# google/ghost-dataplane

Hardware: AMD Instinct MI355X
Metric: Mpkt/s device-resident coprocessor NF pipeline (64B pkts); HBM GB/s vs peak (higher is better)
Workload: dtype u32

## Files before the change

ghost-dataplane_amd/csrc/cop_device.h:

```cpp
#ifndef COP_DEVICE_H
#define COP_DEVICE_H

#include <hip/hip_runtime.h>
#include <stdint.h>

#include "cop_kernels.h"

namespace copd {

constexpr int BLOCK = COPK_BLOCK;
constexpr int WAVES = BLOCK / 64;

typedef uint32_t u32x2 __attribute__((ext_vector_type(2)));
typedef uint32_t u32x4 __attribute__((ext_vector_type(4)));
typedef uint32_t u32x4a __attribute__((ext_vector_type(4), aligned(4)));
typedef uint32_t u32x2a __attribute__((ext_vector_type(2), aligned(4)));

__device__ __forceinline__ uint32_t bswap32(uint32_t x) { return __builtin_bswap32(x); }

__device__ __forceinline__ void lb_store(unsigned long long *p, unsigned long long v)
{
    __hip_atomic_store(p, v, __ATOMIC_RELAXED, __HIP_MEMORY_SCOPE_AGENT);
}

// ... 53 lines not shown
    for (uint32_t q = (uint32_t)wave; q < total; q += WAVES) {
        const bool b1 = q >= f1, b2 = q >= f2, b3 = q >= f3, b4 = q >= f4, b5 = q >= f5;
        const void *g = b5 ? s5.g : b4 ? s4.g : b3 ? s3.g : b2 ? s2.g : b1 ? s1.g : s0.g;
        uint32_t *dst = b5 ? s5.dst : b4 ? s4.dst : b3 ? s3.dst : b2 ? s2.dst : b1 ? s1.dst : s0.dst;
        const uint32_t n16 = b5 ? s5.n16 : b4 ? s4.n16 : b3 ? s3.n16 : b2 ? s2.n16 : b1 ? s1.n16 : s0.n16;
        const uint32_t c = q - (b5 ? f5 : b4 ? f4 : b3 ? f3 : b2 ? f2 : b1 ? f1 : 0u);
        const uint32_t i = c * 64u + (uint32_t)lane;
        if (i < n16)
            __builtin_amdgcn_global_load_lds((const __attribute__((address_space(1))) void *)((const uint4 *)g + i),
                                             (__attribute__((address_space(3))) void *)(dst + c * 256u), 16, 0, 0);
    }
}

__device__ __forceinline__ void lds_stage(uint32_t *lds_dst, const void *gsrc, uint32_t n16, int lane, int wave)
{
    const uint4 *g = (const uint4 *)gsrc;
    for (uint32_t c = (uint32_t)wave; c * 64u < n16; c += WAVES) {
        const uint32_t i = c * 64u + (uint32_t)lane;
        if (i < n16)
            __builtin_amdgcn_global_load_lds((const __attribute__((address_space(1))) void *)(g + i),
                                             (__attribute__((address_space(3))) void *)(lds_dst + c * 256u),
                                             16, 0, 0);
    }
}

__device__ __forceinline__ uint32_t ivt_search(const uint32_t *S, uint32_t m, uint32_t ib, uint32_t lv, uint32_t ip)
{
    const uint16_t *idx = (const uint16_t *)(S + m);
    const uint32_t b = ip >> (32u - ib);
    uint32_t k = idx[b];
    const uint32_t hi = idx[b + 1];
    for (uint32_t step = (1u << lv) >> 1; step; step >>= 1) {
        const uint32_t c = min(k + step, hi);
        if (S[c] <= ip) k = c;
    }
    return k;
}

#ifndef COPK_IVT_VALUE
#define COPK_IVT_VALUE 1
#endif
__device__ __forceinline__ uint32_t ivt_value(const uint32_t *S, const uint32_t *V, uint32_t m, uint32_t ib, uint32_t lv,
                                              uint32_t ip)
{
    if (!COPK_IVT_VALUE || lv == 0) return V[ivt_search(S, m, ib, lv, ip)];
    const uint16_t *idx = (const uint16_t *)(S + m);
    const uint32_t b = ip >> (32u - ib);
    uint32_t k = idx[b];
    const uint32_t hi = idx[b + 1];
    for (uint32_t step = (1u << lv) >> 1; step > 1; step >>= 1) {
        const uint32_t c = min(k + step, hi);
        if (S[c] <= ip) k = c;
    }
    const uint32_t c = min(k + 1, hi);
    const uint32_t sc = S[c], vk = V[k], vc = V[c];
    return sc <= ip ? vc : vk;
}

constexpr int LB_GROUPS = 4;
constexpr uint32_t LB_GAVE_UP = 0xFFFFFFFFu;
__device__ __forceinline__ uint32_t look_back(unsigned long long *chain, uint32_t stride, uint32_t j, uint32_t agg,
                                              uint32_t epoch, uint32_t *err, int lane, const uint32_t *exitw = nullptr,
                                              uint32_t spin_log2 = 22)
{
    const unsigned long long ep = (unsigned long long)epoch << 32;
    if (j == 0) {
        if (lane == 0) lb_store(&chain[0], ep | (2ull << 30) | agg);
        return 0;
    }
    if (lane == 0) lb_store(&chain[(size_t)j * stride], ep | (1ull << 30) | agg);
    uint32_t excl = 0;
    int qhi = (int)j - 1;
    uint32_t spins = 0;
    for (;;) {
        unsigned long long v[LB_GROUPS];
#pragma unroll
        for (int r = 0; r < LB_GROUPS; r++) {
            const int idx = qhi - r * 64 - lane;
            v[r] = idx >= 0 ? lb_load(&chain[(size_t)idx * stride]) : 0ull;
        }
        int consumed = 0;
        bool done = false;
#pragma unroll
        for (int r = 0; r < LB_GROUPS; r++) {
            const bool inb = qhi - r * 64 - lane >= 0;
            const uint32_t flag = (uint32_t)(v[r] >> 30) & 3u;
            const bool ok = inb && (uint32_t)(v[r] >> 32) == epoch && flag != 0u;
            const unsigned long long m_incl = __ballot(ok && flag == 2u);
            const unsigned long long m_bad = __ballot(inb && !ok);
            const int first_incl = m_incl ? __ffsll((long long)m_incl) - 1 : 64;
            const int first_bad = m_bad ? __ffsll((long long)m_bad) - 1 : 64;
            const int upto = min(first_incl + 1, first_bad);
            uint32_t val = lane < upto ? ((uint32_t)v[r] & 0x3FFFFFFFu) : 0u;
#pragma unroll
            for (int off = 32; off; off >>= 1) val += __shfl_xor(val, off);
            excl += val;
            consumed += upto;
            if (first_incl < first_bad) {
                done = true;
                break;
            }
            if (upto < 64) break;
        }
        if (done) break;
        qhi -= consumed;
        if (consumed == 0) {
// ... 157 lines not shown
__device__ __forceinline__ void load_step(const StepGeom &g, const uint8_t *pk0, uint32_t stride, uint32_t pb,
                                          uint32_t last, u32x4 (&v)[3], bool sys = false)
{
    if (sys) {
        const __amdgpu_buffer_rsrc_t rs = sys_rsrc(pk0);
#pragma unroll
        for (int c = 0; c < 3; c++) v[c] = ld_sys16(rs, min(pb + g.lpk[c], last) * stride + g.lch[c]);
        return;
    }
#pragma unroll
    for (int c = 0; c < 3; c++) {
        const uint32_t ic = min(pb + g.lpk[c], last);
        v[c] = __builtin_nontemporal_load((const u32x4 *)(pk0 + (size_t)ic * stride + g.lch[c]));
    }
}

__device__ __forceinline__ void load_step_imix(const StepGeom &g, const uint8_t *pkts, uint32_t off,
                                               uint32_t data_off, u32x4 (&v)[3], bool sys = false)
{
    uint32_t o[3];
#pragma unroll
    for (int c = 0; c < 3; c++)
        o[c] = (uint32_t)__builtin_amdgcn_ds_bpermute((int)(g.lpk[c] << 2), (int)off) + data_off + g.lch[c];
    if (sys) {
        const __amdgpu_buffer_rsrc_t rs = sys_rsrc(pkts);
#pragma unroll
        for (int c = 0; c < 3; c++) v[c] = ld_sys16(rs, o[c]);
        return;
    }
#pragma unroll
    for (int c = 0; c < 3; c++) v[c] = __builtin_nontemporal_load((const u32x4 *)(pkts + o[c]));
}

__device__ __forceinline__ uint32_t load_off_imix(const uint32_t *offsets, uint32_t pb, int lane, uint32_t last,
                                                  bool sys = false)
{
    const uint32_t ic = min(pb + (uint32_t)lane, last);
    return sys ? ld_sys4(sys_rsrc(offsets), ic * 4u) : offsets[ic];
}

__device__ __forceinline__ void gather_step(const StepGeom &g, const u32x4 (&v)[3], uint32_t &w3, uint32_t &w6,
                                            uint32_t &w7, uint32_t &w8)
{
    const uint32_t c0w = g.r3 == 0 ? v[0].w : g.r3 == 1 ? v[2].w : v[1].w;
    const uint32_t c1z = g.r3 == 0 ? v[1].z : g.r3 == 1 ? v[0].z : v[2].z;
    const uint32_t c1w = g.r3 == 0 ? v[1].w : g.r3 == 1 ? v[0].w : v[2].w;
    const uint32_t c2x = g.r3 == 0 ? v[2].x : g.r3 == 1 ? v[1].x : v[0].x;
    w3 = (uint32_t)__builtin_amdgcn_ds_bpermute(g.a3, (int)c0w);
    w6 = (uint32_t)__builtin_amdgcn_ds_bpermute(g.a67, (int)c1z);
    w7 = (uint32_t)__builtin_amdgcn_ds_bpermute(g.a67, (int)c1w);
    w8 = (uint32_t)__builtin_amdgcn_ds_bpermute(g.a8, (int)c2x);
}

struct Opt {
    uint32_t demux;
    uint32_t port_stats;
    uint32_t dbg;
    unsigned long long *rule_hits;
};

__device__ __forceinline__ Opt opt_all(const CopKParams &p)
{
    return Opt{p.demux, p.port_stats, p.dbg, p.rule_hits};
}

struct Tables {
    uint32_t *rt_top;
    uint16_t *rt_leaf;
    uint32_t *fw_s, *fw_v, *lp_s, *lp_v;
};

__device__ __forceinline__ uint32_t probe_ld(const uint32_t *a, uint32_t nt)
{
    return nt ? __builtin_nontemporal_load(a) : *a;
}

__device__ __forceinline__ void bkt_issue(const uint32_t *bidx, uint32_t ib, uint32_t ip, bool reach, uint32_t &k0,
                                          uint32_t &k1)
{
    if (reach) {
        const u32x2a x = *(const u32x2a *)(bidx + (ip >> (32u - ib)));
        k0 = x.x;
        k1 = x.y;
    } else {
        k0 = k1 = 0;
    }
}

template <int FW, int LPM, int PPT>
__device__ __forceinline__ void pass1(const CopKParams &p, const Tables &t, const uint32_t (&w3)[PPT],
                                      const uint32_t (&w6)[PPT], const uint32_t (&w7)[PPT],
                                      const uint32_t (&w8)[PPT], uint32_t (&verdict)[PPT], uint32_t (&port)[PPT],
                                      uint32_t (&src)[PPT], uint32_t (&dst)[PPT], uint32_t (&fwe)[PPT],
                                      uint32_t (&lpe)[PPT], uint32_t (&lpe2)[PPT], uint32_t (&fwe2)[PPT])
{
    const bool stageP = (p.stages & COPK_STAGE_PARSE) != 0;
#pragma unroll
    for (int k = 0; k < PPT; k++) {
        verdict[k] = COPK_FORWARD;
        port[k] = 0;
        const uint32_t et = ((w3[k] & 0xFFu) << 8) | ((w3[k] >> 8) & 0xFFu);
        dst[k] = bswap32(__builtin_amdgcn_alignbit(w8[k], w7[k], 16));
        src[k] = bswap32(__builtin_amdgcn_alignbit(w7[k], w6[k], 16));
        if (stageP) {
            if (et != 0x0800u) {
                verdict[k] = COPK_DROP_PARSE;
                port[k] = 0xFFFFu;
            } else {
                const uint32_t idx = dst[k] & 0xFFFFu;
                const uint32_t top = t.rt_top[idx >> 8];
                port[k] = (top & 0x80000000u) ? (uint32_t)t.rt_leaf[((top & 0xFFFFu) << 8) | (idx & 0xFFu)]
                                              : (top & 0xFFFFu);
                if (port[k] == 0xFFFFu) verdict[k] = COPK_DROP_PARSE;
                else if (port[k] >= p.n_ports) verdict[k] = COPK_DROP_NO_PORT;
            }
        }
        const bool reach = verdict[k] == COPK_FORWARD;
        if (FW == COPK_TBL_IVT) fwe[k] = ivt_value(t.fw_s, t.fw_v, p.fw_m, p.fw_ib, p.fw_lv, src[k]);
        if (FW == COPK_TBL_DIR) fwe[k] = reach ? probe_ld(&p.fw_tbl24[src[k] >> 8], p.probe_nt) : 0u;
        if (FW == COPK_TBL_BKT) bkt_issue(p.fw_bidx, p.fw_ib, src[k], reach, fwe[k], fwe2[k]);
        if (LPM == COPK_TBL_IVT) lpe[k] = ivt_value(t.lp_s, t.lp_v, p.lpm_m, p.lpm_ib, p.lpm_lv, dst[k]);
        if (LPM == COPK_TBL_DIR) lpe[k] = reach ? probe_ld(&p.lpm_tbl24[dst[k] >> 8], p.probe_nt) : 0u;
        if (LPM == COPK_TBL_TRIE) lpe[k] = t.lp_s[dst[k] >> 20];
        if (LPM == COPK_TBL_BKT) bkt_issue(p.lpm_bidx, p.lpm_ib, dst[k], reach, lpe[k], lpe2[k]);
    }
}

template <int PPT>
__device__ __forceinline__ void trie_walk(const uint32_t *nodes, const uint32_t *leaves, const uint32_t (&ip)[PPT],
                                          uint32_t (&e)[PPT], const bool (&live)[PPT])
{
    bool in[PPT], lf[PPT];
    bool any = false;
#pragma unroll
    for (int k = 0; k < PPT; k++) {
        in[k] = live[k] && (e[k] & 0x80000000u);
        lf[k] = false;
        any |= in[k];
    }
#pragma unroll
    for (int l = 0; l < 4; l++) {
        if (!__ballot(any)) break;
        const uint32_t sh = l == 0 ? 14u : l == 1 ? 8u : l == 2 ? 2u : 0u;
        const uint32_t msk = l == 3 ? 3u : 63u;
        u32x4a a[PPT];
        u32x2a b[PPT];
#pragma unroll
        for (int k = 0; k < PPT; k++) {
            if (in[k]) {
                const uint32_t *nd = nodes + (size_t)(e[k] & 0x7FFFFFFFu) * 6u;
                a[k] = *(const u32x4a *)nd;
                b[k] = *(const u32x2a *)(nd + 4);
            }
        }
        any = false;
#pragma unroll
        for (int k = 0; k < PPT; k++) {
            if (in[k]) {
                const uint32_t c = (ip[k] >> sh) & msk;
                const unsigned long long vec = a[k].x | ((unsigned long long)a[k].y << 32);
                const unsigned long long lv = a[k].z | ((unsigned long long)a[k].w << 32);
                const unsigned long long upto = (2ull << c) - 1ull;
                if ((vec >> c) & 1ull) {
                    e[k] = 0x80000000u | (b[k].x + (uint32_t)__popcll(vec & upto) - 1u);
                    any = true;
                } else {
                    e[k] = b[k].y + (uint32_t)__popcll(lv & upto) - 1u;
                    in[k] = false;
                    lf[k] = true;
                }
            }
        }
    }
#pragma unroll
    for (int k = 0; k < PPT; k++)
        if (lf[k]) e[k] = leaves[e[k]];
}

template <int PPT>
__device__ __forceinline__ void tbl8_step(const uint32_t *tbl8, uint32_t packed, const uint32_t (&ip)[PPT],
// ... 676 lines not shown
```

ghost-dataplane_amd/csrc/cop_runtime.cpp:

```cpp
#include <hip/hip_runtime.h>

#include <dlfcn.h>
#include <errno.h>
#include <stdarg.h>
#include <stdio.h>
#include <stdlib.h>
#include <string.h>
#include <time.h>

#include <algorithm>
#include <atomic>
#include <chrono>
#include <condition_variable>
#include <mutex>
#include <thread>
#include <vector>

#include "cop_gpu.h"
#include "cop_internal.h"
#include "cop_kernels.h"
#include <rccl/rccl.h>

namespace {

constexpr uint32_t IVT_MAX = 8192;
constexpr size_t SHARD_WORDS = (size_t)COPK_COUNTER_SHARDS * COP_N_COUNTERS;
constexpr size_t PORT_WORDS = (size_t)COPK_COUNTER_SHARDS * COPK_PORT_WORDS;
constexpr size_t RULE_OFF = SHARD_WORDS + PORT_WORDS;
constexpr uint32_t LOOK_TILE_MIN = COPK_BLOCK;
constexpr int TIMING_SLOTS = 256;
constexpr int MAX_LANES = 4;

struct DevLpm {
    bool loaded = false;
    uint32_t m = 0;
    uint32_t ib = 0, lv = 0, iw = 0;
    uint32_t *starts = nullptr, *vals = nullptr;
    uint32_t *tbl24 = nullptr, *tbl8 = nullptr;
    uint32_t n_ext = 0;
    bool tbl8_packed = false;
    size_t tbl8_bytes = 0;
    uint32_t *tl0 = nullptr, *tnodes = nullptr, *tleaves = nullptr;
    uint32_t t_nodes = 0, t_leaves = 0;
    uint32_t *bidx = nullptr, *bpairs = nullptr;
    uint32_t b_m = 0;
    cop_live_img *img = nullptr;
    uint64_t tab_uid = 0;
    uint32_t grp_cap = 0;
    bool has_table = false;
};

struct LookupStage {
    uint32_t *h = nullptr, *d = nullptr;
    hipEvent_t done = nullptr;
    uint32_t n = 0;
    uint64_t first = 0;
};

constexpr uint32_t LIVE_STAGE_RECS = 65536;
constexpr uint32_t IVT_IW_MAX = ((4096u + 2u) / 2u + 3u) & ~3u;
constexpr uint32_t IVT_STAGE_WORDS = 2 * IVT_MAX + IVT_IW_MAX;
struct LiveStage {
    cop_patch_rec *h = nullptr;
    void *d = nullptr;
    uint32_t *h_ivt = nullptr;
    hipEvent_t copied = nullptr;
    bool used = false;
};

struct Lane {
    hipStream_t s = nullptr;
    unsigned long long *tickets[2] = {nullptr, nullptr};
    uint32_t dirty[2] = {0, 0};
    int parity = 0;
// ... 1500 lines not shown
        L.zc = zc;
        if (zc_in) {
            HIPCHK(c, hipHostMalloc(&L.h_stage, (size_t)batch * COP_HDR16_STRIDE, hipHostMallocMapped));
            void *ds = nullptr;
            HIPCHK(c, hipHostGetDevicePointer(&ds, L.h_stage, 0));
            L.m_stage = (uint8_t *)ds;
        } else {
            HIPCHK(c, hipHostMalloc(&L.h_stage, (size_t)batch * COP_HDR16_STRIDE, hipHostMallocDefault));
            HIPCHK(c, hipMalloc(&L.d_stage, (size_t)batch * COP_HDR16_STRIDE));
        }
        if (zc_out) {
            HIPCHK(c, hipHostMalloc(&L.h_res, (size_t)batch * 8, hipHostMallocMapped));
            void *dr = nullptr;
            HIPCHK(c, hipHostGetDevicePointer(&dr, L.h_res, 0));
            L.m_res = (cop_result *)dr;
        } else {
            HIPCHK(c, hipHostMalloc(&L.h_res, (size_t)batch * 8, hipHostMallocDefault));
            HIPCHK(c, hipMalloc(&L.d_res, (size_t)batch * 8));
        }
        L.cap = batch;
    }
    const uint64_t nb = (n + batch - 1) / batch;
    const bool overlap = c->gather && c->gather->th.size() > 0 && c->n_lanes > 1;
    auto prepare = [&](uint64_t bi, bool async) -> int {
        Lane &L = c->lane[bi % (uint64_t)c->n_lanes];
        const uint64_t first = bi * batch;
        const uint32_t k = (uint32_t)std::min<uint64_t>(batch, n - first);
        const cop_result *prev = nullptr;
        uint32_t prev_n = 0;
        uint64_t prev_first = 0;
        if (L.busy) {
            HIPCHK(c, hipEventSynchronize(L.done));
            L.busy = false;
            prev = L.h_res;
            prev_n = L.n;
            prev_first = L.first;
        }
        cop_result *prev_dst = prev ? results + prev_first : nullptr;
        const size_t prev_bytes = (size_t)prev_n * sizeof(cop_result);
        if (c->gather && async) {
            c->gather->start_async(pkt_data + first, L.h_stage, k, prev, prev_dst, prev_bytes, rec);
        } else if (c->gather) {
            c->gather->run(pkt_data + first, L.h_stage, k, prev, prev_dst, prev_bytes, rec);
        } else {
            if (prev_n) memcpy(prev_dst, prev, prev_bytes);
            GatherPool::slice(pkt_data + first, L.h_stage, k, 1, 0, rec);
        }
        return 0;
    };
    auto issue = [&](uint64_t bi) -> int {
        Lane &L = c->lane[bi % (uint64_t)c->n_lanes];
        const uint64_t first = bi * batch;
        const uint32_t k = (uint32_t)std::min<uint64_t>(batch, n - first);
        if (!zc_in && !(c->dbg & 0x100u))
            HIPCHK(c, hipMemcpyAsync(L.d_stage, L.h_stage, (size_t)k * rec, hipMemcpyHostToDevice, L.s));
        cop_batch b;
        memset(&b, 0, sizeof(b));
        b.pkts = zc_in ? L.m_stage : L.d_stage;
        b.n = k;
        b.stride = rec;
        b.results = zc_out ? L.m_res : L.d_res;
        if (int rc = submit_on(c, L, &b, 1, false, c->cfg.stages)) return rc;
        if (!zc_out) HIPCHK(c, hipMemcpyAsync(L.h_res, L.d_res, (size_t)k * 8, hipMemcpyDeviceToHost, L.s));
        HIPCHK(c, hipEventRecord(L.done, L.s));
        L.busy = true;
        L.first = first;
        L.n = k;
        return 0;
    };
    if (nb)
        if (int rc = prepare(0, false)) return rc;
    for (uint64_t bi = 0; bi < nb; bi++) {
        const bool pre = overlap && bi + 1 < nb;
        if (pre)
            if (int rc = prepare(bi + 1, true)) return rc;
        const int rc = issue(bi);
        if (pre) c->gather->wait();
        if (rc) return rc;
        if (!overlap && bi + 1 < nb)
            if (int rc2 = prepare(bi + 1, false)) return rc2;
    }
    for (int l = 0; l < c->n_lanes; l++)
        if (int rc = lane_finish(c, c->lane[l], results)) return rc;
    if (int rc = take_lane_errors(c, 0xFu)) return rc;
    return 0;
}

static int pmd_hits_flush(cop_ctx *c);
static int pmd_pause(cop_ctx *c);
static int pmd_resume(cop_ctx *c);

static int tele_scratch(cop_ctx *c)
{
    HIPCHK(c, hipSetDevice(c->device));
    if (!c->tele_stream) HIPCHK(c, hipStreamCreateWithFlags(&c->tele_stream, hipStreamNonBlocking));
    const size_t n = RULE_OFF + c->n_rule_ctr;
    if (c->tele_words < n) {
        if (c->tele_dev) (void)hipFree(c->tele_dev);
        c->tele_dev = nullptr;
        c->tele_words = 0;
        HIPCHK(c, hipMalloc(&c->tele_dev, n * 8));
        c->tele_words = n;
    }
    return 0;
}

static int exchange_words(cop_ctx *c, size_t off, size_t n, uint64_t *out, int reset)
// ... 1807 lines not shown
```

ghost-dataplane_amd/csrc/cop_tile.h:

```cpp
#ifndef COP_TILE_H
#define COP_TILE_H

#include "cop_device.h"

namespace copd {

#ifndef COPK_PHASE_STAMPS
#define COPK_PHASE_STAMPS 0
#endif
#define STAMP(ph)                                                                          \
    do {                                                                                   \
        if (((o.dbg & 8u) || (COPK_PHASE_STAMPS && p.stamps)) && tid == 0) {               \
            __builtin_amdgcn_sched_barrier(0);                                             \
            __hip_atomic_store(&p.stamps[blockIdx.x * 8 + (ph)], __builtin_amdgcn_s_memrealtime(), \
                               __ATOMIC_RELAXED, __HIP_MEMORY_SCOPE_AGENT);                     \
            __builtin_amdgcn_sched_barrier(0);                                             \
        }                                                                                  \
    } while (0)

struct LdsCarve {
    Tables tb;
    CompactLds cl;
    uint32_t *s_tile;
    uint32_t *s_red;
// ... 157 lines not shown
#endif
#ifndef COPK_PMD_WIN
#define COPK_PMD_WIN 1
#endif
#ifndef COPK_PMD_WIN_DIR
#define COPK_PMD_WIN_DIR COPK_PMD_WIN
#endif
template <int PPT, int WIN>
constexpr int win_of()
{
    return WIN < PPT ? WIN : PPT;
}
#ifndef COPK_PMD_PRIO
#define COPK_PMD_PRIO 1
#endif
template <int K>
__device__ __forceinline__ void step_prio()
{
    if constexpr (COPK_PMD_PRIO) __builtin_amdgcn_s_setprio(K >= 3 ? 0 : 3 - K);
}
#ifndef COPK_PMD_PRIO_BODY
#define COPK_PMD_PRIO_BODY 0
#endif
template <bool WT, int K>
__device__ __forceinline__ void body_prio()
{
    if constexpr (WT && COPK_PMD_PRIO_BODY) step_prio<K>();
}
#ifndef COPK_PMD_STAGE_LIST
#define COPK_PMD_STAGE_LIST 1
#endif
#ifndef COPK_SEG_WAVE
#define COPK_SEG_WAVE 1
#endif
#ifndef COPK_WAVE_COUNTERS
#define COPK_WAVE_COUNTERS 1
#endif
template <int PPT>
__device__ __forceinline__ uint32_t step_off(int k, int wave)
{
    if constexpr (COPK_SEG_WAVE && PPT == WAVES) return (uint32_t)(wave * PPT * 64 + k * 64);
    else return (uint32_t)(k * BLOCK + wave * 64);
}

template <int PPT, int K0, int K1, int SYS = 2, int WIN = COPK_PMD_WIN>
__device__ __forceinline__ void steps_load(const CopKBatch &B, uint32_t j, int lane, int wave,
                                           u32x4 (&v)[win_of<PPT, WIN>()][3], bool sys_rt = false)
{
    const bool sys = SYS == 2 ? sys_rt : SYS == 1;
    static_assert(K1 <= win_of<PPT, WIN>(), "steps beyond the window");
    const StepGeom sg = step_geom(lane);
    const uint32_t base = j * (BLOCK * PPT);
    const uint32_t last = B.n ? B.n - 1 : 0u;
#pragma unroll
    for (int k = K0; k < K1; k++)
        load_step(sg, B.pkts + B.data_off, B.stride, base + step_off<PPT>(k, wave), last, v[k], sys);
}

template <int FW, int LPM, int PPT, bool WT, int SYS = 2, int WIN = COPK_PMD_WIN,
          bool STAGE_LIST = COPK_PMD_STAGE_LIST, int LAY = COPK_LAY_COALESCED>
__device__ __forceinline__ void tile_steps_v(const CopKParams &p, const LdsCarve &lc, const CopKBatch &B, uint32_t j,
                                             int tid, int lane, int wave, u32x4 (&v)[win_of<PPT, WIN>()][3],
                                             bool sys_rt = false)
{
    const bool sys = SYS == 2 ? sys_rt : SYS == 1;
    static_assert(COPK_SEG == BLOCK, "one segment per tile step");
    const Tables &tb = lc.tb;
    constexpr int TILE = BLOCK * PPT;
    const uint32_t base = j * TILE;
    const uint32_t last = B.n ? B.n - 1 : 0u;
    const StepGeom sg = step_geom(lane);
    constexpr int W = win_of<PPT, WIN>();
    Counts tot;
    uint32_t *r = (uint32_t *)B.results;
    const int i2 = lane & 31;
    const bool staged = STAGE_LIST && B.fwd_idx && lc.cl.stage && !(COPK_XP & 4);
    uint32_t all_prev = 0;
    auto flush = [&](int k, uint32_t len) {
        const uint32_t cc = (uint32_t)wave * 16u + (uint32_t)(lane & 15);
        const uint32_t pk = base + (uint32_t)k * BLOCK;
        if (lane < 16 && cc * 4u < len)
            st_list_chunk<WT>(&lc.cl.stage[k * BLOCK + cc * 4u], B.fwd_idx, pk + cc * 4u, B.n);
    };
    uint32_t run = 0;
    auto emit = [&](int k, bool valid0, uint32_t verdict0, uint32_t flags0, uint32_t port0, uint32_t rnh0) {
        const uint32_t pk0 = base + k * BLOCK;
        const uint32_t wb = base + step_off<PPT>(k, wave);
        const bool valid[1] = {valid0};
        const uint32_t verdict[1] = {verdict0}, flags[1] = {flags0};
        const Counts c = wave_counts<FW, 1>(valid, verdict, flags);
        tot.total += c.total;
        tot.notv4 += c.notv4;
        tot.fwd += c.fwd;
        tot.dropfw += c.dropfw;
        tot.parse += c.parse;
        tot.noport += c.noport;
        tot.rhit += c.rhit;
        tot.rx += c.rx;
        const unsigned long long bal = __ballot(valid0 && verdict0 == COPK_FORWARD);
        if (lane == 0) {
            lc.cl.cnt[k * WAVES + wave] = (uint32_t)__popcll(bal);
            if (k == PPT - 1) {
                const uint32_t c8[8] = {tot.total, tot.notv4, tot.fwd, tot.dropfw, tot.parse, tot.noport, tot.rhit,
                                        tot.rx};
#pragma unroll
                for (int q = 0; q < 8; q++) lc.s_red[wave * 8 + q] = c8[q];
            }
        }
        const uint32_t rx = verdict0 | (flags0 << 8) | (port0 << 16);
        const uint32_t a0 = (uint32_t)__shfl((int)rx, 2 * i2), a1 = (uint32_t)__shfl((int)rnh0, 2 * i2);
        const uint32_t a2 = (uint32_t)__shfl((int)rx, 2 * i2 + 1), a3 = (uint32_t)__shfl((int)rnh0, 2 * i2 + 1);
        const uint32_t idx = wb + 2u * (uint32_t)i2;
        if (lane < 32 && !(COPK_XP & 2)) {
            if (idx + 1 < B.n) st_u32x4<WT>(u32x4{a0, a1, a2, a3}, r, 2 * (long)idx);
            else if (idx < B.n) st_u32x2<WT>(u32x2{a0, a1}, (u32x2 *)&r[2 * (size_t)idx]);
        }
        if (COPK_XP & 4) {
            if (k == PPT - 1) {
                lds_barrier();
                counters_add(p, lc.s_red, tid);
            }
            return;
        }
        if constexpr (COPK_SEG_WAVE && PPT == WAVES) {
            const uint32_t sb = base + (uint32_t)wave * COPK_SEG;
            const uint32_t rank = run + __builtin_amdgcn_mbcnt_hi((uint32_t)(bal >> 32),
                                                                  __builtin_amdgcn_mbcnt_lo((uint32_t)bal, 0u));
            if (staged) {
                if ((bal >> lane) & 1ull) lc.cl.stage[wave * COPK_SEG + rank] = wb + (uint32_t)lane;
            } else if (B.fwd_idx && ((bal >> lane) & 1ull)) {
                st_u32<WT>(wb + (uint32_t)lane, &B.fwd_idx[sb + rank]);
            }
            run += (uint32_t)__popcll(bal);
            if (k == PPT - 1) {
                if (staged) {
                    asm volatile("" ::: "memory");
                    if ((uint32_t)lane * 4u < run)
                        st_list_chunk<WT>(&lc.cl.stage[wave * COPK_SEG + lane * 4], B.fwd_idx, sb + (uint32_t)lane * 4u,
                                          B.n);
                }
                if (B.fwd_count && lane == 0 && sb < B.n) st_u32<WT>(run, B.fwd_count + sb / COPK_SEG);
                if (COPK_WAVE_COUNTERS) {
                    counters_add_wave(p, tot, lane, blockIdx.x * WAVES + (uint32_t)wave);
                } else {
                    lds_barrier();
                    counters_add(p, lc.s_red, tid);
                }
            }
            return;
        }
        lds_barrier();
        uint32_t off = 0, all = 0;
#pragma unroll
        for (int w = 0; w < WAVES; w++) {
            const uint32_t cw = lc.cl.cnt[k * WAVES + w];
            off += w < wave ? cw : 0u;
            all += cw;
        }
        const uint32_t rank = off + __builtin_amdgcn_mbcnt_hi((uint32_t)(bal >> 32),
                                                             __builtin_amdgcn_mbcnt_lo((uint32_t)bal, 0u));
        if (staged) {
            if (k > 0) flush(k - 1, all_prev);
            if ((bal >> lane) & 1ull) lc.cl.stage[k * BLOCK + rank] = pk0 + tid;
            all_prev = all;
        } else if (B.fwd_idx && ((bal >> lane) & 1ull)) {
            st_u32<WT>(pk0 + tid, &B.fwd_idx[pk0 + rank]);
        }
        if (B.fwd_count && tid == 0 && pk0 < B.n) st_u32<WT>(all, B.fwd_count + pk0 / COPK_SEG);
        if (k == PPT - 1) counters_add(p, lc.s_red, tid);
    };
    auto prio = [&](int k) {
        if (COPK_PMD_PRIO) {
            if (k == 0) step_prio<0>();
            else if (k == 1) step_prio<1>();
            else if (k == 2) step_prio<2>();
            else if (k == 3) step_prio<3>();
        }
    };
    if constexpr (LAY == COPK_LAY_IMIX) {
        static_assert((LPM == COPK_TBL_DIR || LPM == COPK_TBL_BKT) && FW != COPK_TBL_DIR && FW != COPK_TBL_BKT,
                      "IMIX steps: DIR-24-8 or bucketed route");
        struct St {
            uint32_t w3, src, dst, verdict, port, fwe, lpe, lpe2;
            bool valid;
            T8 t8;
            BkQ bq;
        };
        St a{}, b{}, c{};
        u32x4 h[3];
        uint32_t off = load_off_imix(B.offsets, base + step_off<PPT>(0, wave), lane, last, sys);
        load_step_imix(sg, B.pkts, off, B.data_off, h, sys);
        if (PPT > 1) off = load_off_imix(B.offsets, base + step_off<PPT>(1, wave), lane, last, sys);
#pragma unroll
        for (int k = 0; k < PPT + 2; k++) {
            if (k < PPT) {
                uint32_t w3[1], w6[1], w7[1], w8[1];
                prio(k);
                gather_step(sg, h, w3[0], w6[0], w7[0], w8[0]);
                uint32_t verdict[1], port[1], fwe[1], lpe[1], lpe2[1], fwe2[1], src[1], dst[1];
                pass1<FW, LPM, 1>(p, tb, w3, w6, w7, w8, verdict, port, src, dst, fwe, lpe, lpe2, fwe2);
                a = St{w3[0], src[0], dst[0], verdict[0], port[0], fwe[0], lpe[0], lpe2[0],
                       base + step_off<PPT>(k, wave) + (uint32_t)lane < B.n && B.n != 0, T8{false, 0ull}, BkQ{}};
                if (k + 1 < PPT) {
                    load_step_imix(sg, B.pkts, off, B.data_off, h, sys);
                    if (k + 2 < PPT) off = load_off_imix(B.offsets, base + step_off<PPT>(k + 2, wave), lane, last, sys);
                }
            }
            if (k >= 1 && k <= PPT) {
                if constexpr (LPM == COPK_TBL_BKT) b.bq = bkt_pairs_issue(p.lpm_bpairs, b.lpe, b.verdict == COPK_FORWARD);
                else b.t8 = tbl8_issue(p.lpm_tbl8, p.lpm_tbl8_packed, b.dst, b.lpe);
            }
            if (k >= 2) {
                const uint32_t w3[1] = {c.w3}, src[1] = {c.src}, dst[1] = {c.dst}, lpe2[1] = {0}, fwe2[1] = {0};
                const bool valid[1] = {c.valid};
                uint32_t verdict[1] = {c.verdict}, fwe[1] = {c.fwe}, flags[1], rnh[1], ct = 0, cn = 0;
                uint32_t lpe[1];
                if constexpr (LPM == COPK_TBL_BKT)
                    lpe[0] = bkt_pairs_finish(p.lpm_bpairs, c.dst, c.lpe, c.lpe2, c.verdict == COPK_FORWARD, c.bq);
                else lpe[0] = tbl8_finish(p.lpm_tbl8, p.lpm_tbl8_packed, c.dst, c.lpe, c.t8);
                pass2<FW, LPM, 1, false>(p, w3, src, dst, valid, fwe, lpe, lpe2, fwe2, verdict, flags, rnh, ct, cn);
                emit(k - 2, valid[0], verdict[0], flags[0], c.port, rnh[0]);
            }
            c = b;
            b = a;
        }
    } else if constexpr (LPM != COPK_TBL_DIR && LPM != COPK_TBL_BKT) {
#pragma unroll
        for (int k = 0; k < PPT; k++) {
            uint32_t w3[1], w6[1], w7[1], w8[1];
            prio(k);
            gather_step(sg, v[k % W], w3[0], w6[0], w7[0], w8[0]);
            if (k + W < PPT)
                load_step(sg, B.pkts + B.data_off, B.stride, base + step_off<PPT>(k + W, wave), last, v[k % W], sys);
            const bool valid[1] = {base + step_off<PPT>(k, wave) + (uint32_t)lane < B.n && B.n != 0};
            uint32_t verdict[1], port[1], flags[1], rnh[1], fwe[1], lpe[1], lpe2[1], fwe2[1], src[1], dst[1], ct = 0,
                cn = 0;
            if (COPK_XP & 1) {
                verdict[0] = (w3[0] ^ w6[0] ^ w7[0] ^ w8[0]) & 1u;
                port[0] = w7[0] & 3u;
                flags[0] = 0;
                rnh[0] = w8[0];
            } else {
                pass1<FW, LPM, 1>(p, tb, w3, w6, w7, w8, verdict, port, src, dst, fwe, lpe, lpe2, fwe2);
                pass2<FW, LPM, 1>(p, w3, src, dst, valid, fwe, lpe, lpe2, fwe2, verdict, flags, rnh, ct, cn);
            }
            emit(k, valid[0], verdict[0], flags[0], port[0], rnh[0]);
        }
    } else {
        static_assert(FW != COPK_TBL_DIR && FW != COPK_TBL_BKT, "firewall lookups in LDS only");
        struct St {
            uint32_t w3, src, dst, verdict, port, fwe, lpe, lpe2;
            bool valid;
            T8 t8;
            BkQ bq;
        };
        St a{}, b{}, c{};
#pragma unroll
        for (int k = 0; k < PPT + 2; k++) {
            if (k < PPT) {
                uint32_t w3[1], w6[1], w7[1], w8[1];
                prio(k);
                gather_step(sg, v[k % W], w3[0], w6[0], w7[0], w8[0]);
                if (k + W < PPT)
                    load_step(sg, B.pkts + B.data_off, B.stride, base + step_off<PPT>(k + W, wave), last, v[k % W],
                              sys);
                uint32_t verdict[1], port[1], fwe[1], lpe[1], lpe2[1], fwe2[1], src[1], dst[1];
                pass1<FW, LPM, 1>(p, tb, w3, w6, w7, w8, verdict, port, src, dst, fwe, lpe, lpe2, fwe2);
                a = St{w3[0], src[0], dst[0], verdict[0], port[0], fwe[0], lpe[0], lpe2[0],
                       base + step_off<PPT>(k, wave) + (uint32_t)lane < B.n && B.n != 0, T8{false, 0ull}, BkQ{}};
            }
            if (k >= 1 && k <= PPT) {
                if constexpr (LPM == COPK_TBL_BKT) b.bq = bkt_pairs_issue(p.lpm_bpairs, b.lpe, b.verdict == COPK_FORWARD);
                else b.t8 = tbl8_issue(p.lpm_tbl8, p.lpm_tbl8_packed, b.dst, b.lpe);
            }
            if (k >= 2) {
                const uint32_t w3[1] = {c.w3}, src[1] = {c.src}, dst[1] = {c.dst}, lpe2[1] = {0}, fwe2[1] = {0};
                const bool valid[1] = {c.valid};
                uint32_t verdict[1] = {c.verdict}, fwe[1] = {c.fwe}, flags[1], rnh[1], ct = 0, cn = 0;
                uint32_t lpe[1];
                if constexpr (LPM == COPK_TBL_BKT)
                    lpe[0] = bkt_pairs_finish(p.lpm_bpairs, c.dst, c.lpe, c.lpe2, c.verdict == COPK_FORWARD, c.bq);
                else lpe[0] = tbl8_finish(p.lpm_tbl8, p.lpm_tbl8_packed, c.dst, c.lpe, c.t8);
                pass2<FW, LPM, 1, false>(p, w3, src, dst, valid, fwe, lpe, lpe2, fwe2, verdict, flags, rnh, ct, cn);
                emit(k - 2, valid[0], verdict[0], flags[0], c.port, rnh[0]);
            }
            c = b;
            b = a;
        }
    }
    if (staged && !(COPK_SEG_WAVE && PPT == WAVES)) {
        lds_barrier();
        flush(PPT - 1, all_prev);
    }
    step_prio<3>();
}

template <int FW, int LPM, int PPT, bool WT, int SYS, int WIN = COPK_PMD_WIN, int LAY = COPK_LAY_COALESCED>
__device__ __forceinline__ void tile_steps(const CopKParams &p, const LdsCarve &lc, const CopKBatch &B, uint32_t j,
                                           int tid, int lane, int wave)
{
    u32x4 v[win_of<PPT, WIN>()][3];
    step_prio<0>();
    if constexpr (LAY != COPK_LAY_IMIX) steps_load<PPT, 0, win_of<PPT, WIN>(), SYS, WIN>(B, j, lane, wave, v);
    tile_steps_v<FW, LPM, PPT, WT, SYS, WIN, COPK_PMD_STAGE_LIST, LAY>(p, lc, B, j, tid, lane, wave, v);
}

template <int FW, int LPM, int LAY, int PPT, bool EXT, bool WT>
__device__ __forceinline__ bool tile_body(const CopKParams &p, const Opt &o, const LdsCarve &lc, const CopKBatch &B,
                                          uint32_t look_off, uint32_t j, const LookCtx &lk, int tid, int lane, int wave,
                                          bool sync_tables, size_t hit_tile, bool sys = false)
{
    constexpr bool IMIX = LAY == COPK_LAY_IMIX;
    const Tables &tb = lc.tb;
    constexpr int TILE = BLOCK * PPT;
    const uint32_t base = j * TILE;
    uint32_t w3[PPT], w6[PPT], w7[PPT], w8[PPT];
    bool valid[PPT];
    const uint32_t last = B.n ? B.n - 1 : 0u;
    if (LAY == COPK_LAY_COALESCED && B.n) {
        const StepGeom sg = step_geom(lane);
// ... 157 lines not shown
```

Measured before the change: 63990.

## Streamline per-step tile kernel: mask selects, scalar pointers, split IVT lookup, lean counters

Replaces the per-step ternary selects with mask-based bit selects, and forces buffer pointers and sizes into scalar registers via readfirstlane. It adds a pass1_step that issues the IVT index loads early and branch-free route computation, and a lean counter path using wave ballots. It also changes the debug-flag gating of the host-to-device copy behind an ablation macro. The intent is to cut VALU/SGPR pressure and hide table-lookup latency, at the cost of more code paths and a changed debug behaviour.

```diff
diff --git a/ghost-dataplane_amd/csrc/cop_device.h b/ghost-dataplane_amd/csrc/cop_device.h
--- a/ghost-dataplane_amd/csrc/cop_device.h
+++ b/ghost-dataplane_amd/csrc/cop_device.h
@@ -129,6 +129,30 @@
         const uint32_t c = min(k + step, hi);
         if (S[c] <= ip) k = c;
     }
+    const uint32_t c = min(k + 1, hi);
+    const uint32_t sc = S[c], vk = V[k], vc = V[c];
+    return sc <= ip ? vc : vk;
+}
+
+struct IvtQ {
+    uint32_t k, hi;
+};
+__device__ __forceinline__ IvtQ ivt_issue(const uint32_t *S, uint32_t m, uint32_t ib, uint32_t ip)
+{
+    const uint16_t *idx = (const uint16_t *)(S + m);
+    const uint32_t b = ip >> (32u - ib);
+    return IvtQ{idx[b], idx[b + 1]};
+}
+__device__ __forceinline__ uint32_t ivt_finish(const uint32_t *S, const uint32_t *V, uint32_t lv, uint32_t ip, IvtQ q)
+{
+    uint32_t k = q.k;
+    const uint32_t hi = q.hi;
+    const uint32_t stop = (COPK_IVT_VALUE && lv != 0) ? 1u : 0u;
+    for (uint32_t step = (1u << lv) >> 1; step > stop; step >>= 1) {
+        const uint32_t c = min(k + step, hi);
+        if (S[c] <= ip) k = c;
+    }
+    if (!stop) return V[k];
     const uint32_t c = min(k + 1, hi);
     const uint32_t sc = S[c], vk = V[k], vc = V[c];
     return sc <= ip ? vc : vk;
@@ -392,6 +416,41 @@
     w8 = (uint32_t)__builtin_amdgcn_ds_bpermute(g.a8, (int)c2x);
 }
 
+struct StepSel {
+    uint32_t m0, m1;
+};
+
+__device__ __forceinline__ StepSel step_sel(const StepGeom &g)
+{
+    StepSel s{g.r3 == 0 ? 0xFFFFFFFFu : 0u, g.r3 == 1 ? 0xFFFFFFFFu : 0u};
+    asm volatile("" : "+v"(s.m0), "+v"(s.m1));
+    return s;
+}
+
+__device__ __forceinline__ uint32_t sel3(const StepSel &s, uint32_t a, uint32_t b, uint32_t c)
+{
+    const uint32_t t = c ^ ((b ^ c) & s.m1);
+    return t ^ ((a ^ t) & s.m0);
+}
+
+__device__ __forceinline__ void gather_step_sel(const StepGeom &g, const StepSel &s, const u32x4 (&v)[3], uint32_t &w3,
+                                                uint32_t &w6, uint32_t &w7, uint32_t &w8)
+{
+    w3 = (uint32_t)__builtin_amdgcn_ds_bpermute(g.a3, (int)sel3(s, v[0].w, v[2].w, v[1].w));
+    w6 = (uint32_t)__builtin_amdgcn_ds_bpermute(g.a67, (int)sel3(s, v[1].z, v[0].z, v[2].z));
+    w7 = (uint32_t)__builtin_amdgcn_ds_bpermute(g.a67, (int)sel3(s, v[1].w, v[0].w, v[2].w));
+    w8 = (uint32_t)__builtin_amdgcn_ds_bpermute(g.a8, (int)sel3(s, v[2].x, v[1].x, v[0].x));
+}
+
+template <typename T>
+__device__ __forceinline__ T *uniform_ptr(T *p)
+{
+    const unsigned long long a = (unsigned long long)p;
+    const uint32_t lo = __builtin_amdgcn_readfirstlane((uint32_t)a);
+    const uint32_t hi = __builtin_amdgcn_readfirstlane((uint32_t)(a >> 32));
+    return (T *)(__attribute__((address_space(1))) T *)(((unsigned long long)hi << 32) | lo);
+}
+
 struct Opt {
     uint32_t demux;
     uint32_t port_stats;
@@ -466,6 +525,45 @@
     }
 }
 
+template <int FW, int LPM>
+__device__ __forceinline__ void pass1_step(const CopKParams &p, const Tables &t, uint32_t w3, uint32_t w6, uint32_t w7,
+                                           uint32_t w8, uint32_t n_ports, uint32_t &verdict, uint32_t &port,
+                                           uint32_t &src, uint32_t &dst, uint32_t &fwe, uint32_t &lpe, uint32_t &lpe2,
+                                           uint32_t &fwe2)
+{
+    const bool stageP = (p.stages & COPK_STAGE_PARSE) != 0;
+    const uint32_t et = ((w3 & 0xFFu) << 8) | ((w3 >> 8) & 0xFFu);
+    dst = bswap32(__builtin_amdgcn_alignbit(w8, w7, 16));
+    src = bswap32(__builtin_amdgcn_alignbit(w7, w6, 16));
+    IvtQ fq{}, lq{};
+    if (FW == COPK_TBL_IVT) fq = ivt_issue(t.fw_s, p.fw_m, p.fw_ib, src);
+    if (LPM == COPK_TBL_IVT) lq = ivt_issue(t.lp_s, p.lpm_m, p.lpm_ib, dst);
+    verdict = COPK_FORWARD;
+    port = 0;
+    uint32_t top = 0, leaf = 0;
+    if (stageP) {
+        const uint32_t idx = dst & 0xFFFFu;
+        top = t.rt_top[idx >> 8];
+        leaf = t.rt_leaf[(top & 0x80000000u) ? ((top & 0xFFFFu) << 8) | (idx & 0xFFu) : 0u];
+    }
+    auto route = [&] {
+        if (!stageP) return;
+        port = ((top & 0x80000000u) ? leaf : (top & 0xFFFFu)) | (et != 0x0800u ? 0xFFFFu : 0u);
+        verdict = port == 0xFFFFu ? COPK_DROP_PARSE : port >= n_ports ? COPK_DROP_NO_PORT : COPK_FORWARD;
+    };
+    constexpr bool probes = FW == COPK_TBL_DIR || FW == COPK_TBL_BKT || LPM == COPK_TBL_DIR || LPM == COPK_TBL_BKT;
+    if (probes) route();
+    const bool reach = verdict == COPK_FORWARD;
+    if (FW == COPK_TBL_IVT) fwe = ivt_finish(t.fw_s, t.fw_v, p.fw_lv, src, fq);
+    if (FW == COPK_TBL_DIR) fwe = reach ? probe_ld(&p.fw_tbl24[src >> 8], p.probe_nt) : 0u;
+    if (FW == COPK_TBL_BKT) bkt_issue(p.fw_bidx, p.fw_ib, src, reach, fwe, fwe2);
+    if (LPM == COPK_TBL_IVT) lpe = ivt_finish(t.lp_s, t.lp_v, p.lpm_lv, dst, lq);
+    if (LPM == COPK_TBL_DIR) lpe = reach ? probe_ld(&p.lpm_tbl24[dst >> 8], p.probe_nt) : 0u;
+    if (LPM == COPK_TBL_TRIE) lpe = t.lp_s[dst >> 20];
+    if (LPM == COPK_TBL_BKT) bkt_issue(p.lpm_bidx, p.lpm_ib, dst, reach, lpe, lpe2);
+    if (!probes) route();
+}
+
 template <int PPT>
 __device__ __forceinline__ void trie_walk(const uint32_t *nodes, const uint32_t *leaves, const uint32_t (&ip)[PPT],
                                           uint32_t (&e)[PPT], const bool (&live)[PPT])
diff --git a/ghost-dataplane_amd/csrc/cop_runtime.cpp b/ghost-dataplane_amd/csrc/cop_runtime.cpp
--- a/ghost-dataplane_amd/csrc/cop_runtime.cpp
+++ b/ghost-dataplane_amd/csrc/cop_runtime.cpp
@@ -20,6 +20,10 @@
 #include "cop_internal.h"
 #include "cop_kernels.h"
 #include <rccl/rccl.h>
+
+#ifndef COP_STREAM_ABLATION
+#define COP_STREAM_ABLATION 0
+#endif
 
 namespace {
 
@@ -1626,7 +1630,7 @@
         Lane &L = c->lane[bi % (uint64_t)c->n_lanes];
         const uint64_t first = bi * batch;
         const uint32_t k = (uint32_t)std::min<uint64_t>(batch, n - first);
-        if (!zc_in && !(c->dbg & 0x100u))
+        if (!zc_in && !(COP_STREAM_ABLATION && (c->dbg & 0x100u)))
             HIPCHK(c, hipMemcpyAsync(L.d_stage, L.h_stage, (size_t)k * rec, hipMemcpyHostToDevice, L.s));
         cop_batch b;
         memset(&b, 0, sizeof(b));
diff --git a/ghost-dataplane_amd/csrc/cop_tile.h b/ghost-dataplane_amd/csrc/cop_tile.h
--- a/ghost-dataplane_amd/csrc/cop_tile.h
+++ b/ghost-dataplane_amd/csrc/cop_tile.h
@@ -233,9 +233,10 @@
     const StepGeom sg = step_geom(lane);
     const uint32_t base = j * (BLOCK * PPT);
     const uint32_t last = B.n ? B.n - 1 : 0u;
-#pragma unroll
-    for (int k = K0; k < K1; k++)
-        load_step(sg, B.pkts + B.data_off, B.stride, base + step_off<PPT>(k, wave), last, v[k], sys);
+    const uint8_t *const pk0 = uniform_ptr(B.pkts + B.data_off);
+    const uint32_t stride0 = __builtin_amdgcn_readfirstlane(B.stride);
+#pragma unroll
+    for (int k = K0; k < K1; k++) load_step(sg, pk0, stride0, base + step_off<PPT>(k, wave), last, v[k], sys);
 }
 
 template <int FW, int LPM, int PPT, bool WT, int SYS = 2, int WIN = COPK_PMD_WIN,
@@ -251,11 +252,21 @@
     const uint32_t base = j * TILE;
     const uint32_t last = B.n ? B.n - 1 : 0u;
     const StepGeom sg = step_geom(lane);
+    const StepSel ss = step_sel(sg);
     constexpr int W = win_of<PPT, WIN>();
     Counts tot;
-    uint32_t *r = (uint32_t *)B.results;
+    uint32_t *r = uniform_ptr((uint32_t *)B.results);
+    uint32_t *const fidx = uniform_ptr(B.fwd_idx);
+    uint32_t *const fcnt = uniform_ptr(B.fwd_count);
+    const uint32_t bn = __builtin_amdgcn_readfirstlane(B.n);
+    const uint8_t *const pk0 = uniform_ptr(B.pkts + B.data_off);
+    const uint32_t stride0 = __builtin_amdgcn_readfirstlane(B.stride);
+    uint32_t nports = p.n_ports;
+    asm volatile("" : "+v"(nports));
     const int i2 = lane & 31;
-    const bool staged = STAGE_LIST && B.fwd_idx && lc.cl.stage && !(COPK_XP & 4);
+    constexpr bool LEAN = COPK_SEG_WAVE && PPT == WAVES && COPK_WAVE_COUNTERS && !(COPK_XP & 4);
+    uint32_t n_parse = 0, n_noport = 0, n_notv4 = 0, n_rhit = 0;
+    const bool staged = STAGE_LIST && fidx && lc.cl.stage && !(COPK_XP & 4);
     uint32_t all_prev = 0;
     auto flush = [&](int k, uint32_t len) {
         const uint32_t cc = (uint32_t)wave * 16u + (uint32_t)(lane & 15);
@@ -267,25 +278,35 @@
     auto emit = [&](int k, bool valid0, uint32_t verdict0, uint32_t flags0, uint32_t port0, uint32_t rnh0) {
         const uint32_t pk0 = base + k * BLOCK;
         const uint32_t wb = base + step_off<PPT>(k, wave);
-        const bool valid[1] = {valid0};
-        const uint32_t verdict[1] = {verdict0}, flags[1] = {flags0};
-        const Counts c = wave_counts<FW, 1>(valid, verdict, flags);
-        tot.total += c.total;
-        tot.notv4 += c.notv4;
-        tot.fwd += c.fwd;
-        tot.dropfw += c.dropfw;
-        tot.parse += c.parse;
-        tot.noport += c.noport;
-        tot.rhit += c.rhit;
-        tot.rx += c.rx;
-        const unsigned long long bal = __ballot(valid0 && verdict0 == COPK_FORWARD);
-        if (lane == 0) {
-            lc.cl.cnt[k * WAVES + wave] = (uint32_t)__popcll(bal);
-            if (k == PPT - 1) {
-                const uint32_t c8[8] = {tot.total, tot.notv4, tot.fwd, tot.dropfw, tot.parse, tot.noport, tot.rhit,
-                                        tot.rx};
-#pragma unroll
-                for (int q = 0; q < 8; q++) lc.s_red[wave * 8 + q] = c8[q];
+        const bool fwd0 = valid0 && verdict0 == COPK_FORWARD;
+        const unsigned long long bal = __ballot(fwd0);
+        if constexpr (LEAN) {
+            const uint32_t vv = valid0 ? verdict0 : (uint32_t)COPK_FORWARD;
+            n_parse += (uint32_t)__popcll(__ballot(vv == COPK_DROP_PARSE));
+            n_noport += (uint32_t)__popcll(__ballot(vv == COPK_DROP_NO_PORT));
+            if (FW != COPK_TBL_OFF) n_notv4 += (uint32_t)__popcll(__ballot(vv == COPK_DROP_NOT_IPV4));
+            if (LPM != COPK_TBL_OFF) n_rhit += (uint32_t)__popcll(__ballot(valid0 && (flags0 & COPK_FLAG_ROUTE_HIT)));
+            asm volatile("" : "+s"(n_parse), "+s"(n_noport), "+s"(n_notv4), "+s"(n_rhit));
+        } else {
+            const bool valid[1] = {valid0};
+            const uint32_t verdict[1] = {verdict0}, flags[1] = {flags0};
+            const Counts c = wave_counts<FW, 1>(valid, verdict, flags);
+            tot.total += c.total;
+            tot.notv4 += c.notv4;
+            tot.fwd += c.fwd;
+            tot.dropfw += c.dropfw;
+            tot.parse += c.parse;
+            tot.noport += c.noport;
+            tot.rhit += c.rhit;
+            tot.rx += c.rx;
+            if (lane == 0) {
+                lc.cl.cnt[k * WAVES + wave] = (uint32_t)__popcll(bal);
+                if (k == PPT - 1) {
+                    const uint32_t c8[8] = {tot.total, tot.notv4, tot.fwd, tot.dropfw, tot.parse, tot.noport, tot.rhit,
+                                            tot.rx};
+#pragma unroll
+                    for (int q = 0; q < 8; q++) lc.s_red[wave * 8 + q] = c8[q];
+                }
             }
         }
         const uint32_t rx = verdict0 | (flags0 << 8) | (port0 << 16);
@@ -293,8 +314,8 @@
         const uint32_t a2 = (uint32_t)__shfl((int)rx, 2 * i2 + 1), a3 = (uint32_t)__shfl((int)rnh0, 2 * i2 + 1);
         const uint32_t idx = wb + 2u * (uint32_t)i2;
         if (lane < 32 && !(COPK_XP & 2)) {
-            if (idx + 1 < B.n) st_u32x4<WT>(u32x4{a0, a1, a2, a3}, r, 2 * (long)idx);
-            else if (idx < B.n) st_u32x2<WT>(u32x2{a0, a1}, (u32x2 *)&r[2 * (size_t)idx]);
+            if (idx + 1 < bn) st_u32x4<WT>(u32x4{a0, a1, a2, a3}, r, 2 * (long)idx);
+            else if (idx < bn) st_u32x2<WT>(u32x2{a0, a1}, (u32x2 *)&r[2 * (size_t)idx]);
         }
         if (COPK_XP & 4) {
             if (k == PPT - 1) {
@@ -308,19 +329,28 @@
             const uint32_t rank = run + __builtin_amdgcn_mbcnt_hi((uint32_t)(bal >> 32),
                                                                   __builtin_amdgcn_mbcnt_lo((uint32_t)bal, 0u));
             if (staged) {
-                if ((bal >> lane) & 1ull) lc.cl.stage[wave * COPK_SEG + rank] = wb + (uint32_t)lane;
-            } else if (B.fwd_idx && ((bal >> lane) & 1ull)) {
-                st_u32<WT>(wb + (uint32_t)lane, &B.fwd_idx[sb + rank]);
+                if (fwd0) lc.cl.stage[wave * COPK_SEG + rank] = wb + (uint32_t)lane;
+            } else if (fidx && fwd0) {
+                st_u32<WT>(wb + (uint32_t)lane, &fidx[sb + rank]);
             }
             run += (uint32_t)__popcll(bal);
             if (k == PPT - 1) {
                 if (staged) {
                     asm volatile("" ::: "memory");
                     if ((uint32_t)lane * 4u < run)
-                        st_list_chunk<WT>(&lc.cl.stage[wave * COPK_SEG + lane * 4], B.fwd_idx, sb + (uint32_t)lane * 4u,
-                                          B.n);
+                        st_list_chunk<WT>(&lc.cl.stage[wave * COPK_SEG + lane * 4], fidx, sb + (uint32_t)lane * 4u, bn);
                 }
-                if (B.fwd_count && lane == 0 && sb < B.n) st_u32<WT>(run, B.fwd_count + sb / COPK_SEG);
+                if (fcnt && lane == 0 && sb < bn) st_u32<WT>(run, fcnt + sb / COPK_SEG);
+                if constexpr (LEAN) {
+                    tot.rx = bn > sb ? min(bn - sb, (uint32_t)COPK_SEG) : 0u;
+                    tot.fwd = run;
+                    tot.parse = n_parse;
+                    tot.noport = n_noport;
+                    tot.notv4 = n_notv4;
+                    tot.rhit = n_rhit;
+                    tot.total = FW != COPK_TBL_OFF ? tot.rx - n_parse - n_noport : 0u;
+                    tot.dropfw = tot.rx - run - n_parse - n_noport - n_notv4;
+                }
                 if (COPK_WAVE_COUNTERS) {
                     counters_add_wave(p, tot, lane, blockIdx.x * WAVES + (uint32_t)wave);
                 } else {
@@ -377,9 +407,10 @@
             if (k < PPT) {
                 uint32_t w3[1], w6[1], w7[1], w8[1];
                 prio(k);
-                gather_step(sg, h, w3[0], w6[0], w7[0], w8[0]);
+                gather_step_sel(sg, ss, h, w3[0], w6[0], w7[0], w8[0]);
                 uint32_t verdict[1], port[1], fwe[1], lpe[1], lpe2[1], fwe2[1], src[1], dst[1];
-                pass1<FW, LPM, 1>(p, tb, w3, w6, w7, w8, verdict, port, src, dst, fwe, lpe, lpe2, fwe2);
+                pass1_step<FW, LPM>(p, tb, w3[0], w6[0], w7[0], w8[0], nports, verdict[0], port[0], src[0], dst[0], fwe[0], lpe[0],
+                                    lpe2[0], fwe2[0]);
                 a = St{w3[0], src[0], dst[0], verdict[0], port[0], fwe[0], lpe[0], lpe2[0],
                        base + step_off<PPT>(k, wave) + (uint32_t)lane < B.n && B.n != 0, T8{false, 0ull}, BkQ{}};
                 if (k + 1 < PPT) {
@@ -410,9 +441,9 @@
         for (int k = 0; k < PPT; k++) {
             uint32_t w3[1], w6[1], w7[1], w8[1];
             prio(k);
-            gather_step(sg, v[k % W], w3[0], w6[0], w7[0], w8[0]);
+            gather_step_sel(sg, ss, v[k % W], w3[0], w6[0], w7[0], w8[0]);
             if (k + W < PPT)
-                load_step(sg, B.pkts + B.data_off, B.stride, base + step_off<PPT>(k + W, wave), last, v[k % W], sys);
+                load_step(sg, pk0, stride0, base + step_off<PPT>(k + W, wave), last, v[k % W], sys);
             const bool valid[1] = {base + step_off<PPT>(k, wave) + (uint32_t)lane < B.n && B.n != 0};
             uint32_t verdict[1], port[1], flags[1], rnh[1], fwe[1], lpe[1], lpe2[1], fwe2[1], src[1], dst[1], ct = 0,
                 cn = 0;
@@ -422,7 +453,8 @@
                 flags[0] = 0;
                 rnh[0] = w8[0];
             } else {
-                pass1<FW, LPM, 1>(p, tb, w3, w6, w7, w8, verdict, port, src, dst, fwe, lpe, lpe2, fwe2);
+                pass1_step<FW, LPM>(p, tb, w3[0], w6[0], w7[0], w8[0], nports, verdict[0], port[0], src[0], dst[0], fwe[0], lpe[0],
+                                    lpe2[0], fwe2[0]);
                 pass2<FW, LPM, 1>(p, w3, src, dst, valid, fwe, lpe, lpe2, fwe2, verdict, flags, rnh, ct, cn);
             }
             emit(k, valid[0], verdict[0], flags[0], port[0], rnh[0]);
@@ -441,12 +473,12 @@
             if (k < PPT) {
                 uint32_t w3[1], w6[1], w7[1], w8[1];
                 prio(k);
-                gather_step(sg, v[k % W], w3[0], w6[0], w7[0], w8[0]);
+                gather_step_sel(sg, ss, v[k % W], w3[0], w6[0], w7[0], w8[0]);
                 if (k + W < PPT)
-                    load_step(sg, B.pkts + B.data_off, B.stride, base + step_off<PPT>(k + W, wave), last, v[k % W],
-                              sys);
+                    load_step(sg, pk0, stride0, base + step_off<PPT>(k + W, wave), last, v[k % W], sys);
                 uint32_t verdict[1], port[1], fwe[1], lpe[1], lpe2[1], fwe2[1], src[1], dst[1];
-                pass1<FW, LPM, 1>(p, tb, w3, w6, w7, w8, verdict, port, src, dst, fwe, lpe, lpe2, fwe2);
+                pass1_step<FW, LPM>(p, tb, w3[0], w6[0], w7[0], w8[0], nports, verdict[0], port[0], src[0], dst[0], fwe[0], lpe[0],
+                                    lpe2[0], fwe2[0]);
                 a = St{w3[0], src[0], dst[0], verdict[0], port[0], fwe[0], lpe[0], lpe2[0],
                        base + step_off<PPT>(k, wave) + (uint32_t)lane < B.n && B.n != 0, T8{false, 0ull}, BkQ{}};
             }
```

Result: no change. 63140 (median of 2 runs) (-1.3%).
